# IseanB/SensorFusion-KalmanFilter

Hardware: AMD Instinct MI355X
Metric: KF predict+update steps/sec (batched filters) (higher is better)
Workload: dtype f64

## Files before the change

### include/kf.h

```cpp
#ifndef KFMI_KF_H
#define KFMI_KF_H

#include <stdint.h>

#ifdef __cplusplus
extern "C" {
#endif

#define KF_OK        0
#define KF_EINVAL   (-1)
#define KF_EHIP     (-2)
#define KF_ENOTSPD  (-3)
#define KF_ENODEV   (-4)
#define KF_ENOMEM   (-5)

#define KF_F32 0
#define KF_F64 1

#define KF_MODEL_CV2 2
#define KF_MODEL_CV3 3

#define KF_MODEL_REF15 15

#define KF_MODEL_REF8 8
// ... 76 lines not shown

int kf_run_events(kf_batch* handle, int T, const uint8_t* etype, const double* dt, const void* payload,
                  void* traj, void* cov, void* logdet, uint8_t* updated, int gate, double threshold,
                  void* stream);

int kf_run_events_seq(kf_batch* handle, int T, const uint8_t* etype, const double* dt, const void* payload,
                      void* traj, void* cov, void* logdet, uint8_t* updated, int gate, double threshold,
                      void* stream);

int kf_run_events_gates(kf_batch* handle, int T, const uint8_t* etype, const double* dt, const void* payload,
                        void* traj, void* cov, void* logdet, uint8_t* updated, const double* thresholds,
                        void* stream);

int kf_run_stream(kf_batch* handle, int T, const uint8_t* etype, const double* dt, const void* payload,
                  void* traj, void* cov, void* logdet, uint8_t* updated, int chunk, int warmup,
                  void* stream);

int kf_run_sweep(kf_batch* handle, int T, const uint8_t* etype, const double* dt, const void* payload,
                 const double* thresholds, void* traj, void* logdet, uint8_t* updated, int32_t* n_updated,
                 int ckpt_every, void* ckpt_x, void* ckpt_P, void* stream);

int kf_stream_check(kf_batch* handle, double* out, void* stream);

int kf_eval_combos(kf_batch* handle, int n_events, const double* events, const double* init,
                   double prev_time, double target_end, int k, uint64_t combo_offset, void* logdets,
                   void* max_logdet, int32_t* n_records, void* stream);

int kf_search_combos(kf_batch* handle, int n_events, const double* events, const double* init,
                     double prev_time, double target_end, double threshold, int k_max, int exhaustive,
                     int n_fixed, uint64_t fixed_mask, uint64_t* winner, int* k_found,
                     uint64_t* n_accepted, void* subset_max, void* stream);

int kf_search_windows(kf_batch* handle, int W, int n_max, const int32_t* n_events, const double* events,
                      const double* init, const double* prev_time, const double* target_end,
                      const double* threshold, int k_max, uint64_t* winner, int32_t* k_found,
                      uint64_t* n_accepted, void* stream);

int kf_search_plan(const kf_batch* handle, int n_events, const double* init, int n_fixed, uint64_t fixed_mask,
                   int k_max, int64_t* out);

int kf_search_info(const kf_batch* handle, int64_t* out);

int kf_score_candidates(kf_batch* handle, int n_types, const int32_t* types, int full, void* gain,
                        void* post, void* stream);

int kf_score_rows(kf_batch* handle, int n_cand, const int32_t* types, const uint32_t* row_masks, void* gain,
// ... 58 lines not shown
```

### sensorfusion-kalmanfilter_amd/csrc/kf_capi.cpp

```cpp
#include <hip/hip_runtime.h>

#include <algorithm>
#include <cmath>
#include <climits>
#include <cstdarg>
#include <cstdlib>
#include <cstdio>
#include <cstring>
#include <mutex>
#include <string>
#include <vector>

#include "../../include/kf.h"
#include "kf_internal.h"

struct kf_batch {
    int model;
    int axes;
    int n, m, c;
    int np;
    int dtype;
    int64_t B;
    int device;
    kf_params params;
// ... 47 lines not shown

thread_local std::string g_err;

int fail(int code, const char* fmt, ...) __attribute__((format(printf, 2, 3)));
int fail(int code, const char* fmt, ...) {
    char buf[512];
    va_list ap;
    va_start(ap, fmt);
    vsnprintf(buf, sizeof buf, fmt, ap);
    va_end(ap);
    g_err = buf;
    return code;
}

int hip_fail(hipError_t e, const char* what) {
    return fail(KF_EHIP, "%s: %s (%d)", what, hipGetErrorString(e), static_cast<int>(e));
}

size_t elem(const kf_batch* h) { return h->dtype == KF_F64 ? 8 : 4; }
int64_t ntri(const kf_batch* h) { return h->np; }

constexpr int kMaxComboEvents = 64;
constexpr int64_t kChainMaxFilters = 16384;
constexpr size_t kWsEvents = sizeof(double) * kMaxComboEvents * 11;
constexpr size_t kWsBinom = sizeof(uint64_t) * (kMaxComboEvents + 1) * (kMaxComboEvents + 1);
constexpr size_t kWsInit = sizeof(double) * 42;
constexpr uint64_t kSearchChildMajorParents = 200000;
constexpr uint64_t kSearchHeadSteps = 400000;
constexpr uint64_t kSearchEndSteps = 200000;
constexpr uint64_t kSearchPairParents = uint64_t(1) << 22;

int64_t opt(const kf_batch* h, int o) { return h->opt[o]; }

bool is_ref15(const kf_batch* h) { return h->model == KF_MODEL_REF15; }

const uint64_t* binom_table() {
    static uint64_t binom[(kMaxComboEvents + 1) * (kMaxComboEvents + 1)];
    static std::once_flag once;
    std::call_once(once, [] {
        for (int a = 0; a <= kMaxComboEvents; ++a)
            for (int b = 0; b <= kMaxComboEvents; ++b) {
                uint64_t v = 0;
                if (b == 0) v = 1;
                else if (a > 0 && b <= a) v = binom[(a - 1) * (kMaxComboEvents + 1) + b - 1] + binom[(a - 1) * (kMaxComboEvents + 1) + b];
                binom[a * (kMaxComboEvents + 1) + b] = v;
            }
// ... 625 lines not shown
    if (int rc = need_cv(h, "kf_synth")) return rc;
    if (T < 0 || update_every < 1 || filter_offset < 0)
        return fail(KF_EINVAL, "kf_synth: bad T/update_every/filter_offset");
    if (h->B && (!x0_out || (T > 0 && !u_out) || (T / update_every > 0 && !z_out)))
        return fail(KF_EINVAL, "kf_synth: null output stream");
    if (h->B == 0) return KF_OK;
    kfmi::SynthArgs a{};
    a.B = h->B;
    a.filter_offset = filter_offset;
    a.seed = seed;
    a.T = T;
    a.update_every = update_every;
    a.dt = dt;
    a.x0 = x0_out;
    a.u = u_out;
    a.z = z_out;
    hipError_t e = kfmi::launch_synth(h->axes, h->dtype == KF_F64, a, static_cast<hipStream_t>(stream));
    if (e != hipSuccess) return hip_fail(e, "kf_synth");
    return KF_OK;
}

namespace {

int run_events_launch(kf_batch* h, int T, const uint8_t* etype, const double* dt, const void* payload, void* traj,
                      void* cov, void* logdet, uint8_t* updated, int gate, double threshold, const int32_t* skip,
                      void* stream, int forced = -1, const double* thresholds = nullptr) {
    kfmi::RefArgs a = ref_args(h);
    a.thresholds = thresholds;
    a.T = T;
    a.etype = etype;
    a.dt = dt;
    a.payload = payload;
    a.traj = traj;
    a.cov = cov;
    a.logdet = logdet;
    a.updated = updated;
    a.gate = gate;
    a.threshold = threshold;
    a.skip = skip;
    const uint64_t span = static_cast<uint64_t>(h->B) * elem(h);
    const bool chain_ok = span * 27u < (uint64_t(1) << 32);
    const bool lds_ok = h->B % 16 == 0 && span * 9u < (uint64_t(1) << 32);
    int variant = h->B < kChainMaxFilters && chain_ok ? kfmi::kEventsChain
                  : lds_ok                            ? kfmi::kEventsLds
                                                      : kfmi::kEventsLane;
    const int64_t v = opt(h, KF_OPT_EVENTS_KERNEL);
    if (v == 2 && chain_ok) variant = kfmi::kEventsChain;
    else if (v == 1) variant = kfmi::kEventsLane;
    else if (v == 3 && lds_ok) variant = kfmi::kEventsLds;
    else if (v == 4 && h->B == 1 && gate && h->dtype == KF_F64) variant = kfmi::kEventsGated;
    if (forced >= 0) variant = forced;
    if (skip && variant != kfmi::kEventsChain && variant != kfmi::kEventsGated)
        return fail(KF_EINVAL, "kf_run_stream: fallback needs the chain kernel");
    hipError_t e = kfmi::launch_ref_events(h->model, h->dtype == KF_F64, a, static_cast<hipStream_t>(stream), variant);
    return e == hipSuccess ? KF_OK : hip_fail(e, "kf_run_events");
}

constexpr int kStreamMinEvents = 65536;
constexpr int kStreamGateWarmup = 2048;
constexpr int kStreamLookaheadShare = 8;
constexpr int64_t kStreamLftEvents = 2048;
constexpr int kStreamPolish = 0;
constexpr int64_t kStreamLftPiece = 160;
constexpr int64_t kStreamTargetChunks = 8192;
constexpr int64_t kStreamMinChunk = 32;
constexpr int64_t kStreamStartLdsMaps = 65536 / (36 * 8);
#ifndef KF_START_MAX_G
#define KF_START_MAX_G 2
#endif

size_t align256(size_t n) { return (n + 255) & ~size_t(255); }

}

namespace {
// ... 262 lines not shown
    } else {
        if (e == hipSuccess) e = chain(C, sa.mx, sa.mP, sa.mst, L, 0, false, nullptr, 1, 4);
        for (int ph : {kfmi::kStreamPhaseScanTiles, kfmi::kStreamPhaseTop, kfmi::kStreamPhaseStarts})
            if (e == hipSuccess && (ph != kfmi::kStreamPhaseTop || top))
                e = kfmi::launch_stream_phase(h->model, f64, ph, sa, st);
        if (e == hipSuccess) e = chain(C, sa.fx, sa.fP, sa.fst, L, 0, true);
        if (e == hipSuccess) e = kfmi::launch_stream_phase(h->model, f64, kfmi::kStreamPhaseFinish, sa, st);
    }
    if (e != hipSuccess) return hip_fail(e, "kf_run_stream");
    if (gate && f64 && updated && opt(h, KF_OPT_EVENTS_KERNEL) == 0) {
        e = kfmi::launch_stream_choose(sa.check, updated, T, kStreamLookaheadShare, st);
        if (e != hipSuccess) return hip_fail(e, "kf_run_stream");
        int rc = run_events_launch(h, T, etype, dt, payload, traj, cov, logdet, updated, gate, threshold,
                                   &sa.check->skip_gated, stream, kfmi::kEventsGated);
        if (rc != KF_OK) return rc;
        return run_events_launch(h, T, etype, dt, payload, traj, cov, logdet, updated, gate, threshold,
                                 &sa.check->skip_chain, stream, kfmi::kEventsChain);
    }
    return run_events_launch(h, T, etype, dt, payload, traj, cov, logdet, updated, gate, threshold, &sa.check->ok,
                             stream);
}
}

int kf_stream_check(kf_batch* h, double* out, void* stream) {
    if (int rc = check_handle(h)) return rc;
    if (!out) return fail(KF_EINVAL, "kf_stream_check: null output");
    if (!h->stream_ws && h->s_chunks != 1) return fail(KF_EINVAL, "kf_stream_check: no kf_run_stream on this handle");
    kfmi::StreamCheck k{};
    if (h->s_chunks > 1) {
        hipError_t e = hipMemcpyAsync(&k, h->stream_ws, sizeof k, hipMemcpyDeviceToHost, static_cast<hipStream_t>(stream));
        if (e == hipSuccess) e = hipStreamSynchronize(static_cast<hipStream_t>(stream));
        if (e != hipSuccess) return hip_fail(e, "kf_stream_check");
    }
    out[0] = k.ok;
    out[1] = (k.bad & ~kfmi::kStreamBadStart) ? 1.0 : 0.0;
    out[2] = k.cov_gap;
    out[3] = k.state_gap;
    out[4] = double(h->s_chunks);
    out[5] = double(h->s_len);
    out[6] = double(h->s_warm);
    out[7] = h->s_chunks > 1 && k.ok ? 0.0 : k.skip_chain ? 4.0 : 2.0;
    return KF_OK;
}

int kf_eval_combos(kf_batch* h, int n_events, const double* events, const double* init, double prev_time,
                   double target_end, int k, uint64_t combo_offset, void* logdets, void* max_logdet,
// ... 636 lines not shown
```

### sensorfusion-kalmanfilter_amd/csrc/kf_common.h

```cpp
#pragma once

#include <hip/hip_runtime.h>
#include <math.h>
#include <stdint.h>

namespace kfmi {
namespace dev {

constexpr int32_t kNotSpd = -3;

template <int N>
__host__ __device__ constexpr int tri(int i, int j) {
    return i <= j ? i * N - i * (i - 1) / 2 + (j - i) : j * N - j * (j - 1) / 2 + (i - j);
}

__device__ __forceinline__ double fmaT(double a, double b, double c) { return __builtin_fma(a, b, c); }
__device__ __forceinline__ float fmaT(float a, float b, float c) { return __builtin_fmaf(a, b, c); }

template <typename T>
__device__ __forceinline__ T quiet_nan();
template <>
__device__ __forceinline__ double quiet_nan<double>() { return __builtin_nan(""); }
template <>
__device__ __forceinline__ float quiet_nan<float>() { return __builtin_nanf(""); }
// ... 91 lines not shown
template <typename T>
__device__ __forceinline__ void det2(const T (&P)[3], T& num, bool& ok) {
    const T m2 = fmaT(-P[1], P[1], P[0] * P[2]);
    ok = ok && (P[0] > T(0)) && (m2 > T(0));
    num *= m2;
}
template <typename T>
__device__ __forceinline__ void renorm(T& prod, int& ex) {
    int e;
    prod = frexp(prod, &e);
    ex += e;
}

template <int N, typename T>
__device__ __forceinline__ T logdet_ldl(const T (&P)[N * (N + 1) / 2]) {
    T prod = T(1);
    int ex = 0;
    bool ok = true;
    ldl_pivot_product<N, T>(P, prod, ex, ok);
    const T ld = log_mant(prod, ex);
    return ok ? ld : quiet_nan<T>();
}

template <int N, int M, bool DIAG_R, typename T, int NEWTON = 2, bool POISON = true, int NV = 1, bool JOSEPH = true,
          bool GAIN_R = false>
__device__ __forceinline__ bool sel_update_nv(T (&xv)[NV][N], T (&P)[N * (N + 1) / 2], const T (&zv)[NV][M],
                                              const T (&R)[M * (M + 1) / 2]) {
    constexpr int MT = M * (M + 1) / 2;
    T S[MT];
#pragma unroll
    for (int i = 0; i < M; ++i)
#pragma unroll
        for (int j = i; j < M; ++j)
            S[tri<M>(i, j)] = (i == j || !DIAG_R) ? P[tri<N>(i, j)] + R[tri<M>(i, j)] : P[tri<N>(i, j)];
    T L[M][M];
    T d[M];
    T dinv[M];
    bool ok = true;
#pragma unroll
    for (int j = 0; j < M; ++j) {
        T v[M];
        T dj = S[tri<M>(j, j)];
#pragma unroll
        for (int k = 0; k < j; ++k) {
            v[k] = L[j][k] * d[k];
            dj = fmaT(-L[j][k], v[k], dj);
        }
        ok = ok && (dj > T(0));
        d[j] = dj;
        dinv[j] = POISON ? rcp_pos<NEWTON>(dj) : rcp_nr<NEWTON>(dj);
#pragma unroll
        for (int i = j + 1; i < M; ++i) {
            T s = S[tri<M>(i, j)];
#pragma unroll
            for (int k = 0; k < j; ++k) s = fmaT(-L[i][k], v[k], s);
            L[i][j] = s * dinv[j];
        }
    }
    T K[N][M];
#pragma unroll
    for (int i = 0; i < N; ++i) {
        T w[M];
#pragma unroll
        for (int a = 0; a < M; ++a) {
            T s = P[tri<N>(i, a)];
#pragma unroll
            for (int b = 0; b < a; ++b) s = fmaT(-L[a][b], w[b], s);
            w[a] = s;
        }
#pragma unroll
        for (int a = M - 1; a >= 0; --a) {
            T s = w[a] * dinv[a];
#pragma unroll
            for (int b = a + 1; b < M; ++b) s = fmaT(-L[b][a], K[i][b], s);
            K[i][a] = s;
        }
    }
#pragma unroll
    for (int v = 0; v < NV; ++v) {
        T y[M];
#pragma unroll
        for (int a = 0; a < M; ++a) y[a] = zv[v][a] - xv[v][a];
#pragma unroll
        for (int i = 0; i < N; ++i) {
            T s = xv[v][i];
#pragma unroll
            for (int a = 0; a < M; ++a) s = fmaT(K[i][a], y[a], s);
            xv[v][i] = s;
        }
    }
    if constexpr (GAIN_R && M == N && DIAG_R) {
#pragma unroll
        for (int i = 0; i < N; ++i)
#pragma unroll
            for (int j = i; j < N; ++j) P[tri<N>(i, j)] = K[i][j] * R[tri<M>(j, j)];
        return ok;
    }
    T top[M][N];
#pragma unroll
    for (int i = 0; i < N; ++i) {
        T E[M];
        if constexpr (JOSEPH) {
#pragma unroll
            for (int a = 0; a < M; ++a) {
                T e = -P[tri<N>(i, a)];
#pragma unroll
                for (int b = 0; b < M; ++b) e = fmaT(K[i][b], S[tri<M>(b, a)], e);
                E[a] = e;
            }
        }
#pragma unroll
        for (int j = i; j < N; ++j) {
            T s = P[tri<N>(i, j)];
#pragma unroll
            for (int b = 0; b < M; ++b) s = fmaT(-K[i][b], P[tri<N>(b, j)], s);
            if constexpr (JOSEPH) {
#pragma unroll
                for (int a = 0; a < M; ++a) s = fmaT(E[a], K[j][a], s);
            }
            if (i < M)
                top[i][j] = s;
            else
                P[tri<N>(i, j)] = s;
        }
    }
#pragma unroll
    for (int i = 0; i < M; ++i)
#pragma unroll
        for (int j = i; j < N; ++j) P[tri<N>(i, j)] = top[i][j];
    return ok;
}

template <int N, int M, bool DIAG_R, typename T, int NEWTON = 2, bool POISON = true, bool JOSEPH = true,
          bool GAIN_R = false>
__device__ __forceinline__ bool sel_update(T (&x)[N], T (&P)[N * (N + 1) / 2], const T (&z)[M],
                                           const T (&R)[M * (M + 1) / 2]) {
    T xv[1][N], zv[1][M];
#pragma unroll
    for (int i = 0; i < N; ++i) xv[0][i] = x[i];
#pragma unroll
    for (int a = 0; a < M; ++a) zv[0][a] = z[a];
    const bool ok = sel_update_nv<N, M, DIAG_R, T, NEWTON, POISON, 1, JOSEPH, GAIN_R>(xv, P, zv, R);
#pragma unroll
    for (int i = 0; i < N; ++i) x[i] = xv[0][i];
    return ok;
}

typedef unsigned int v2u __attribute__((ext_vector_type(2)));

__device__ __forceinline__ __amdgpu_buffer_rsrc_t row_rsrc(const void* base, int64_t r, uint32_t row_bytes) {
    const char* p = reinterpret_cast<const char*>(base) + r * int64_t(row_bytes);
    return __builtin_amdgcn_make_buffer_rsrc(const_cast<char*>(p), 0, row_bytes, 0x00020000);
}
// ... 131 lines not shown
```

### sensorfusion-kalmanfilter_amd/csrc/kf_internal.h

```cpp
#pragma once

#include <hip/hip_runtime.h>
#include <stdint.h>

namespace kfmi {

struct CvArgs {
    int64_t B;
    int T;
    int update_every;
    double dt;
    const double* dt_steps;
    const double* dt_filter;
    void* x;
    void* P;
    int32_t* status;
    const void* u;
    const void* x0;
    const void* z;
    const uint8_t* mask;
    void* traj;
    void* logdet;
    double q_pos, q_vel;
    double r[6];
// ... 254 lines not shown
    int gps_wins;
    bool fused;
    int group_waves;
    bool one_launch;
    uint32_t* wave_key;
    uint32_t* wave_id;
    uint32_t* wave_key_sorted;
    uint32_t* order;
    void* sort_tmp;
    size_t sort_tmp_bytes;
    const uint32_t* words;
    int n_words;
    int32_t* words_used;
    bool rec_time;
};

enum class Op { Run, Predict, Update, Step, Reset };

hipError_t launch_cv(int axes, bool f64, Op op, const CvArgs& a, hipStream_t stream);
hipError_t launch_cv_offblock(int axes, bool f64, const CvArgs& a, int* flag, hipStream_t stream);
hipError_t launch_synth(int axes, bool f64, const SynthArgs& a, hipStream_t stream);
hipError_t launch_copy(void* dst, const void* src, size_t bytes, hipStream_t stream);
constexpr int kEventsLane = 0, kEventsChain = 1, kEventsLds = 2, kEventsGated = 3;
hipError_t launch_ref_events(int model, bool f64, const RefArgs& a, hipStream_t stream, int variant);
hipError_t launch_ref_stream(int model, bool f64, const RefArgs& a, hipStream_t stream, int nv = 1);
hipError_t launch_ref_sweep(int model, bool f64, const SweepArgs& a, hipStream_t stream);
hipError_t launch_ref_reset(int model, bool f64, const RefArgs& a, hipStream_t stream);
hipError_t launch_ref15_combos(bool f64, const Ref15ComboArgs& a, hipStream_t stream);
hipError_t launch_ref15_search(bool f64, const Ref15SearchArgs& a, bool child_major, hipStream_t stream);
hipError_t launch_ref15_search_pair(bool f64, const Ref15SearchArgs& a, bool child_major, hipStream_t stream);
void set_search_band(Ref15SearchArgs& a, bool f64);
hipError_t launch_ref15_search_head(bool f64, const Ref15SearchArgs& a, hipStream_t stream);
hipError_t launch_ref15_search_end(bool f64, const Ref15SearchArgs& a, hipStream_t stream);
hipError_t launch_ref15_search_windows(bool f64, bool sym, const Ref15WindowArgs* wins, int W, uint64_t max_lanes,
                                       int n_max, int k_max, const uint64_t* binom, const RefConsts* kc,
                                       hipStream_t stream);
hipError_t launch_search_windows_finish(const Ref15WindowArgs* wins, int W, int k_max, uint64_t* host,
                                        hipStream_t stream);
hipError_t launch_search_finish(uint64_t* counters, uint64_t* host, int n, bool zero, hipStream_t stream);
hipError_t launch_ref15_score(bool f64, const Ref15ScoreArgs& a, hipStream_t stream);
hipError_t launch_ref15_scheduled(bool f64, const Ref15SchedArgs& a, hipStream_t stream);
hipError_t launch_ref15_random_picks(const Ref15SchedArgs& a, int32_t* pick, hipStream_t stream);
hipError_t sort_pairs_desc_u32(void* tmp, size_t* tmp_bytes, const uint32_t* keys_in, uint32_t* keys_out,
                               const uint32_t* vals_in, uint32_t* vals_out, int n, int bits, hipStream_t stream);

constexpr int kBlock = 256;
// ... 5 lines not shown
```

### sensorfusion-kalmanfilter_amd/csrc/kf_ref.hip

```cpp
#include <hip/hip_runtime.h>
#include <stdint.h>

#include <cmath>
#include <cstdlib>
#include <cstring>

#include "kf_common.h"
#include "kf_internal.h"

namespace kfmi {
namespace {

template <typename T>
__device__ __forceinline__ __attribute__((address_space(4))) const T* ro(const T* p) {
    return (__attribute__((address_space(4))) const T*)p;
}
typedef __attribute__((address_space(4))) const double ro_double;
typedef __attribute__((address_space(4))) const uint64_t ro_u64;

using namespace dev;

constexpr int kGps = 0, kImu = 1;
constexpr int kRefNewton = 1;
#ifndef KF_REF_JOSEPH_F64
#define KF_REF_JOSEPH_F64 0
#endif
template <typename T>
constexpr bool kRefJoseph = sizeof(T) == 4 || KF_REF_JOSEPH_F64 != 0;
// ... 941 lines not shown
                    gap = fmax(gap, fabs(pe - wnx[k]));
                }
                const double rel = gap / fmax(scale, 1e-300);
                crel = rel == rel ? rel : __builtin_inf();
            }
        }
        if (a.s_check) {
            crel = fmax(crel, dpp_d<kDppXor1>(crel));
            crel = fmax(crel, dpp_d<kDppXor2>(crel));
            crel = fmax(crel, dpp_d<kDppHalfMirror>(crel));
            const bool full = (g & ~int64_t(63)) / LPF + 64 / LPF <= a.B;
            if (full) {
#pragma unroll
                for (int sh = kGroup; sh < 64; sh <<= 1) crel = fmax(crel, __shfl_xor(crel, sh, 64));
                const bool lane0 = (threadIdx.x & 63) == 0;
                if (lane0 && crel != 0.0) atomic_max_pos(&a.s_check->cov_gap, crel);
                const bool any_bad = __builtin_amdgcn_ballot_w64(c == 0 && st != 0) != 0;
                if (lane0 && any_bad) atomicOr(&a.s_check->bad, kStreamBadFilter);
            } else {
                if (c == 0 && vb == 0 && crel != 0.0) atomic_max_pos(&a.s_check->cov_gap, crel);
                if (c == 0 && vb == 0 && st != 0) atomicOr(&a.s_check->bad, kStreamBadFilter);
            }
        }
    }
}

#ifndef KF_SWEEP_DEPTH
#define KF_SWEEP_DEPTH 4
#endif
constexpr int kSweepDepth = KF_SWEEP_DEPTH;
constexpr int kSweepBlock = 64;

template <typename T, class M, bool CUSTOM>
__global__ __launch_bounds__(kSweepBlock) void ref_sweep_kernel(const SweepArgs a) {
    const int64_t g = static_cast<int64_t>(blockIdx.x) * kSweepBlock + threadIdx.x;
    const int64_t f = g / kGroup;
    if (f >= a.B) return;
    const int c = static_cast<int>(g % kGroup);
    const bool pva = c < M::NP;
    const bool live = c < M::NP + M::NA;
    const int ca = pva ? c : (live ? c - M::NP : 0);
    const uint32_t off = uint32_t(f) * uint32_t(sizeof(T));
    const uint32_t rb = uint32_t(a.B) * uint32_t(sizeof(T));
    int xi[3], pr[6];
#pragma unroll
    for (int k = 0; k < 3; ++k) xi[k] = !live ? -1 : pva ? M::pva(ca, k) : (k < 2 ? M::aw(ca, k) : -1);
// ... 2970 lines not shown
    KF_CUSTOM_DISPATCH(a.kc, {
        if (lds) {
            if (f64) ref15_sched_lds_kernel<double, CUSTOM><<<grid, kBlock, 0, stream>>>(a);
            else ref15_sched_lds_kernel<float, CUSTOM><<<grid, kBlock, 0, stream>>>(a);
        } else {
            if (f64) ref15_sched_kernel<double, CUSTOM><<<grid, kBlock, 0, stream>>>(a);
            else ref15_sched_kernel<float, CUSTOM><<<grid, kBlock, 0, stream>>>(a);
        }
    });
    return hipGetLastError();
}

namespace {
template <typename T, class M, bool CUSTOM>
void ref_events_t(const RefArgs& a, hipStream_t stream, int variant) {
    if (a.thresholds) {
        if (variant == kEventsLds) {
            const dim3 grid(static_cast<unsigned>((a.B + kBlock - 1) / kBlock));
            if (a.cov) ref_events_lds_kernel<T, M, true, CUSTOM, true><<<grid, kBlock, 0, stream>>>(a);
            else ref_events_lds_kernel<T, M, false, CUSTOM, true><<<grid, kBlock, 0, stream>>>(a);
        } else if (variant == kEventsChain) {
            const dim3 cgrid(static_cast<unsigned>((a.B * kGroup + kBlock - 1) / kBlock));
            ref_chain_kernel<T, M, false, CUSTOM, 1, true><<<cgrid, kBlock, 0, stream>>>(a);
        } else {
            const dim3 grid(static_cast<unsigned>((a.B + kBlock - 1) / kBlock));
            ref_events_kernel<T, M, CUSTOM, true><<<grid, kBlock, 0, stream>>>(a);
        }
        return;
    }
    if (variant == kEventsLds) {
        const dim3 grid(static_cast<unsigned>((a.B + kBlock - 1) / kBlock));
        if (a.cov) ref_events_lds_kernel<T, M, true, CUSTOM><<<grid, kBlock, 0, stream>>>(a);
        else ref_events_lds_kernel<T, M, false, CUSTOM><<<grid, kBlock, 0, stream>>>(a);
    } else if (variant == kEventsChain) {
        const dim3 cgrid(static_cast<unsigned>((a.B * kGroup + kBlock - 1) / kBlock));
        ref_chain_kernel<T, M, false, CUSTOM><<<cgrid, kBlock, 0, stream>>>(a);
    } else if (variant == kEventsGated) {
        ref_chain_gated_kernel<T, M, CUSTOM><<<1, 64, 0, stream>>>(a);
    } else {
        const dim3 grid(static_cast<unsigned>((a.B + kBlock - 1) / kBlock));
        ref_events_kernel<T, M, CUSTOM><<<grid, kBlock, 0, stream>>>(a);
    }
}
template <typename T, class M, bool CUSTOM>
void ref_stream_t(const RefArgs& a, hipStream_t stream, int nv) {
    if (nv == 4) {
        const dim3 vgrid(static_cast<unsigned>((a.B * chain_lanes<4>() + kBlock - 1) / kBlock));
        ref_chain_kernel<T, M, true, CUSTOM, 4><<<vgrid, kBlock, 0, stream>>>(a);
    } else {
        const dim3 cgrid(static_cast<unsigned>((a.B * kGroup + kBlock - 1) / kBlock));
        ref_chain_kernel<T, M, true, CUSTOM><<<cgrid, kBlock, 0, stream>>>(a);
    }
}
}

hipError_t launch_ref_events(int model, bool f64, const RefArgs& a, hipStream_t stream, int variant) {
    if (model != 15 && model != 8) return hipErrorInvalidValue;
    if (a.thresholds && (variant == kEventsGated || a.s_len != 0)) return hipErrorInvalidValue;
    KF_CUSTOM_DISPATCH(a.kc, {
// ... 349 lines not shown
```

### sensorfusion-kalmanfilter_amd/kfmi/_lib.py

```python
from __future__ import annotations

import ctypes
import glob
import hashlib
import os
import re

HERE = os.path.dirname(os.path.abspath(__file__))
LIB_PATH = os.path.abspath(os.environ.get('KFMI_LIB') or os.path.join(HERE, 'libkfmi.so'))
HEADER = os.path.normpath(os.path.join(HERE, '..', '..', 'include', 'kf.h'))
CSRC = os.path.normpath(os.path.join(HERE, '..', 'csrc'))

KF_OK = 0
KF_EINVAL = -1
KF_EHIP = -2
KF_ENOTSPD = -3
KF_ENODEV = -4
KF_ENOMEM = -5
KF_F32 = 0
KF_F64 = 1
KF_MODEL_CV2 = 2
KF_MODEL_CV3 = 3
KF_MODEL_REF15 = 15
KF_MODEL_REF8 = 8
# ... 63 lines not shown
    'kf_last_error': (ctypes.c_char_p, []),
    'kf_default_params': (_i, [_i, ctypes.POINTER(kf_params)]),
    'kf_device_count': (_i, [ctypes.POINTER(_i)]),
    'kf_init': (_i, [_i]),
    'kf_alloc': (_i, [ctypes.POINTER(_vp), _i, _i64, _i, ctypes.POINTER(kf_params)]),
    'kf_free': (_i, [_vp]),
    'kf_release_retired': (_i, [_vp, ctypes.POINTER(_i64)]),
    'kf_dims': (_i, [_vp, ctypes.POINTER(_i), ctypes.POINTER(_i), ctypes.POINTER(_i),
                     ctypes.POINTER(_i64), ctypes.POINTER(_i)]),
    'kf_reset': (_i, [_vp, _vp, _vp]),
    'kf_set_state': (_i, [_vp, _vp, _vp, _i, _vp]),
    'kf_get_state': (_i, [_vp, _vp, _vp, _i, _vp]),
    'kf_get_status': (_i, [_vp, _vp, _i, _vp]),
    'kf_predict': (_i, [_vp, _d, _vp, _vp, _vp, _vp]),
    'kf_update': (_i, [_vp, _vp, _vp, _vp, _vp]),
    'kf_run': (_i, [_vp, _i, _d, _vp, _vp, _vp, _vp, _i, _vp, _vp, _vp]),
    'kf_synth': (_i, [_vp, ctypes.c_uint64, _i64, _i, _d, _i, _vp, _vp, _vp, _vp]),
    'kf_run_events': (_i, [_vp, _i, _vp, _vp, _vp, _vp, _vp, _vp, _vp, _i, _d, _vp]),
    'kf_run_events_seq': (_i, [_vp, _i, _vp, _vp, _vp, _vp, _vp, _vp, _vp, _i, _d, _vp]),
    'kf_run_events_gates': (_i, [_vp, _i, _vp, _vp, _vp, _vp, _vp, _vp, _vp, _vp, _vp]),
    'kf_run_stream': (_i, [_vp, _i, _vp, _vp, _vp, _vp, _vp, _vp, _vp, _i, _i, _vp]),
    'kf_run_sweep': (_i, [_vp, _i, _vp, _vp, _vp, _vp, _vp, _vp, _vp, _vp, _i, _vp, _vp, _vp]),
    'kf_stream_check': (_i, [_vp, _vp, _vp]),
    'kf_eval_combos': (_i, [_vp, _i, _vp, _vp, _d, _d, _i, ctypes.c_uint64, _vp, _vp, _vp, _vp]),
    'kf_search_combos': (_i, [_vp, _i, _vp, _vp, _d, _d, _d, _i, _i, _i, ctypes.c_uint64,
                              ctypes.POINTER(ctypes.c_uint64), ctypes.POINTER(_i), _vp, _vp, _vp]),
    'kf_search_windows': (_i, [_vp, _i, _i, _vp, _vp, _vp, _vp, _vp, _vp, _i, _vp, _vp, _vp, _vp]),
    'kf_search_plan': (_i, [_vp, _i, _vp, _i, ctypes.c_uint64, _i, _vp]),
    'kf_search_info': (_i, [_vp, _vp]),
    'kf_score_candidates': (_i, [_vp, _i, _vp, _i, _vp, _vp, _vp]),
    'kf_score_rows': (_i, [_vp, _i, _vp, _vp, _vp, _vp, _vp]),
    'kf_run_scheduled': (_i, [_vp, _i, _vp, _vp, _vp, _vp, _vp, _d, _vp, _vp, _vp, _vp, _vp]),
    'kf_run_scheduled_rec': (_i, [_vp, _i, _vp, _vp, _vp, _i, _vp, _vp, _d, _vp, _vp, _vp, _vp, _vp]),
    'kf_run_scheduled_random': (_i, [_vp, _i, _vp, _vp, _vp, _i, _vp, _vp, _d, _vp, _i, _vp, _vp, _vp, _vp, _vp,
                                     _vp]),
    'kf_sched_random_picks': (_i, [_vp, _i, _vp, _vp, _vp, _vp, _d, _vp, _i, _vp, _vp, _vp, _vp, _vp]),
    'kf_csv_shape': (_i, [ctypes.c_char_p, _i, ctypes.POINTER(_i64), ctypes.POINTER(_i)]),
    'kf_csv_read': (_i, [ctypes.c_char_p, _i, _i, _vp, _i64, _i64]),
    'kf_ingest': (_i, [_vp, _i64, _i64, _vp, _i64, _i64, _i, _vp, _vp, _vp, _vp, _vp, _vp, _vp,
                       ctypes.POINTER(kf_ingest_info), _vp]),
    'kf_quat_to_euler': (_i, [_i64, _vp, _i64, _vp, _vp]),
    'kf_events_dt': (_i, [_i64, _vp, _vp, _d, _i, _vp, _vp, _vp]),
    'kf_events_select': (_i, [_i64, _vp, _vp, _vp, _i, _vp, _vp, _vp, ctypes.POINTER(_i64), _vp]),
}

_lib = None
# ... 71 lines not shown
```

### sensorfusion-kalmanfilter_amd/kfmi/engine.py

```python
from __future__ import annotations

import ctypes

import numpy as np
import torch

from . import _lib
from ._lib import KFError, check

MODELS = {
    'cv2': (_lib.KF_MODEL_CV2, 4, 2, 2, 10),
    'cv3': (_lib.KF_MODEL_CV3, 6, 3, 3, 21),
    'ref15': (_lib.KF_MODEL_REF15, 15, 3, 0, 27),
    'ref8': (_lib.KF_MODEL_REF8, 8, 2, 0, 15),
}
REF_MODELS = ('ref15', 'ref8')
TRAJ_WIDTH = {'ref15': 6, 'ref8': 3}
DTYPES = {'f32': (_lib.KF_F32, torch.float32, np.float32), 'f64': (_lib.KF_F64, torch.float64, np.float64)}


OPTIONS = {
    'predict': (_lib.KF_OPT_PREDICT, {'auto': 0, 'deferred': 0, 'eager': 1}),
    'cv_kernel': (_lib.KF_OPT_CV_KERNEL, {'auto': 0, 'general': 1, 'block2': 2, 'block4': 4, 'block8': 8}),
    'blocks_per_cu': (_lib.KF_OPT_BLOCKS_PER_CU, {'auto': 0}),
# ... 319 lines not shown
                  checkpoint_every=0):
        if self.model not in REF_MODELS:
            raise ValueError('run_sweep needs a ref15 or ref8 handle')
        T = int(etype.shape[0])
        every = int(checkpoint_every)
        if every < 0:
            raise ValueError('checkpoint_every must be >= 0')
        et = self._dev(etype.reshape(T), (T,), 'etype', torch.uint8)
        dtd = self._dev(dt.reshape(T), (T,), 'dt', torch.float64)
        pay = self._dev(payload.reshape(T, 9), (T, 9), 'payload')
        thr = self._dev(thresholds, (self.batch,), 'thresholds', torch.float64)
        tr = self.empty(T, TRAJ_WIDTH[self.model], self.batch) if traj else None
        ld = self.empty(T, self.batch) if logdet else None
        up = torch.empty(T, self.batch, dtype=torch.uint8, device=self.device) if updated else None
        nu = torch.zeros(self.batch, dtype=torch.int32, device=self.device) if counts else None
        C = T // every if every > 0 else 0
        cx = self.empty(C, self.n, self.batch) if every > 0 else None
        cP = self.empty(C, self.ntri, self.batch) if every > 0 else None
        check(_lib.lib().kf_run_sweep(self.handle, T, _ptr(et), _ptr(dtd), _ptr(pay), _ptr(thr), _ptr(tr), _ptr(ld),
                                      _ptr(up), _ptr(nu), every, _ptr(cx) if C else None, _ptr(cP) if C else None,
                                      self._stream()))
        return tr, ld, up, nu, cx, cP

    def stream_check(self):
        out = (ctypes.c_double * 8)()
        check(_lib.lib().kf_stream_check(self.handle, out, self._stream()))
        return dict(ok=bool(out[0]), failed_chunk=bool(out[1]), cov_gap=out[2], state_gap=out[3],
                    chunks=int(out[4]), chunk=int(out[5]), warmup=int(out[6]),
                    fallback={0: None, 2: 'chain', 4: 'gated'}[int(out[7])])

    def eval_combos(self, events, init, prev_time, target_end, k, combo_offset=0, logdets=True):
        if self.model != 'ref15':
            raise ValueError('eval_combos needs a ref15 handle')
        ev = np.ascontiguousarray(events, dtype=np.float64)
        ini = np.ascontiguousarray(init, dtype=np.float64)
        if ev.ndim != 2 or ev.shape[1] != 11 or ini.shape != (42,):
            raise ValueError('events must be [n, 11] and init [42]')
        mx = self.empty(self.batch)
        ld = self.empty(k + 2, self.batch) if logdets else None
        nr = torch.empty(self.batch, dtype=torch.int32, device=self.device)
        check(_lib.lib().kf_eval_combos(self.handle, ev.shape[0], ev.ctypes.data_as(ctypes.c_void_p),
                                        ini.ctypes.data_as(ctypes.c_void_p), float(prev_time), float(target_end),
                                        int(k), int(combo_offset), _ptr(ld), _ptr(mx), _ptr(nr), self._stream()))
        torch.cuda.current_stream(self.device).synchronize()
        return mx, ld, nr

# ... 187 lines not shown
```

Baseline: 57.45 billion.

## Add warp-specialized split chain kernel for small-batch event runs

Adds a new events kernel for batches of up to 4096 filters. One wave runs the covariance predict and gain computation, a second wave applies the gains to the state and writes the records, and an optional third wave computes log-determinants. The waves hand gains and covariances to each other through double-buffered LDS in batches of events, so the serial covariance chain overlaps with state updates and output stores. This costs block-wide barriers per batch, 64 KB of static LDS per block, and fewer filters per block. The headline metric is for batched filters and may run at a batch size that never reaches this path.

```diff
diff --git a/include/kf.h b/include/kf.h
--- a/include/kf.h
+++ b/include/kf.h
@@ -122,6 +122,8 @@
 
 int kf_stream_check(kf_batch* handle, double* out, void* stream);
 
+int kf_events_kernel(const kf_batch* handle, int gate, int* kernel);
+
 int kf_eval_combos(kf_batch* handle, int n_events, const double* events, const double* init,
                    double prev_time, double target_end, int k, uint64_t combo_offset, void* logdets,
                    void* max_logdet, int32_t* n_records, void* stream);
diff --git a/sensorfusion-kalmanfilter_amd/csrc/kf_capi.cpp b/sensorfusion-kalmanfilter_amd/csrc/kf_capi.cpp
--- a/sensorfusion-kalmanfilter_amd/csrc/kf_capi.cpp
+++ b/sensorfusion-kalmanfilter_amd/csrc/kf_capi.cpp
@@ -93,6 +93,7 @@
 
 constexpr int kMaxComboEvents = 64;
 constexpr int64_t kChainMaxFilters = 16384;
+constexpr int64_t kSplitMaxFilters = 4096;
 constexpr size_t kWsEvents = sizeof(double) * kMaxComboEvents * 11;
 constexpr size_t kWsBinom = sizeof(uint64_t) * (kMaxComboEvents + 1) * (kMaxComboEvents + 1);
 constexpr size_t kWsInit = sizeof(double) * 42;
@@ -764,6 +765,23 @@
 
 namespace {
 
+int events_variant(const kf_batch* h, int gate, int forced) {
+    const uint64_t span = static_cast<uint64_t>(h->B) * elem(h);
+    const bool chain_ok = span * 27u < (uint64_t(1) << 32);
+    const bool lds_ok = h->B % 16 == 0 && span * 9u < (uint64_t(1) << 32);
+    int variant = h->B < kChainMaxFilters && chain_ok ? kfmi::kEventsChain
+                  : lds_ok                            ? kfmi::kEventsLds
+                                                      : kfmi::kEventsLane;
+    const int64_t v = opt(h, KF_OPT_EVENTS_KERNEL);
+    if (v == 2 && chain_ok) variant = kfmi::kEventsChain;
+    else if (v == 1) variant = kfmi::kEventsLane;
+    else if (v == 3 && lds_ok) variant = kfmi::kEventsLds;
+    else if (v == 4 && h->B == 1 && gate && h->dtype == KF_F64) variant = kfmi::kEventsGated;
+    if (forced >= 0) variant = forced;
+    if (v != 2 && variant == kfmi::kEventsChain && h->B <= kSplitMaxFilters) variant = kfmi::kEventsSplit;
+    return variant;
+}
+
 int run_events_launch(kf_batch* h, int T, const uint8_t* etype, const double* dt, const void* payload, void* traj,
                       void* cov, void* logdet, uint8_t* updated, int gate, double threshold, const int32_t* skip,
                       void* stream, int forced = -1, const double* thresholds = nullptr) {
@@ -780,19 +798,8 @@
     a.gate = gate;
     a.threshold = threshold;
     a.skip = skip;
-    const uint64_t span = static_cast<uint64_t>(h->B) * elem(h);
-    const bool chain_ok = span * 27u < (uint64_t(1) << 32);
-    const bool lds_ok = h->B % 16 == 0 && span * 9u < (uint64_t(1) << 32);
-    int variant = h->B < kChainMaxFilters && chain_ok ? kfmi::kEventsChain
-                  : lds_ok                            ? kfmi::kEventsLds
-                                                      : kfmi::kEventsLane;
-    const int64_t v = opt(h, KF_OPT_EVENTS_KERNEL);
-    if (v == 2 && chain_ok) variant = kfmi::kEventsChain;
-    else if (v == 1) variant = kfmi::kEventsLane;
-    else if (v == 3 && lds_ok) variant = kfmi::kEventsLds;
-    else if (v == 4 && h->B == 1 && gate && h->dtype == KF_F64) variant = kfmi::kEventsGated;
-    if (forced >= 0) variant = forced;
-    if (skip && variant != kfmi::kEventsChain && variant != kfmi::kEventsGated)
+    const int variant = events_variant(h, gate, forced);
+    if (skip && variant != kfmi::kEventsChain && variant != kfmi::kEventsSplit && variant != kfmi::kEventsGated)
         return fail(KF_EINVAL, "kf_run_stream: fallback needs the chain kernel");
     hipError_t e = kfmi::launch_ref_events(h->model, h->dtype == KF_F64, a, static_cast<hipStream_t>(stream), variant);
     return e == hipSuccess ? KF_OK : hip_fail(e, "kf_run_events");
@@ -1101,6 +1108,20 @@
 }
 }
 
+int kf_events_kernel(const kf_batch* h, int gate, int* kernel) {
+    if (int rc = check_handle(h)) return rc;
+    if (!is_ref(h)) return fail(KF_EINVAL, "kf_events_kernel: needs a KF_MODEL_REF15 or KF_MODEL_REF8 handle");
+    if (!kernel) return fail(KF_EINVAL, "kf_events_kernel: null output");
+    switch (events_variant(h, gate, -1)) {
+        case kfmi::kEventsLane: *kernel = 1; break;
+        case kfmi::kEventsChain: *kernel = 2; break;
+        case kfmi::kEventsLds: *kernel = 3; break;
+        case kfmi::kEventsGated: *kernel = 4; break;
+        default: *kernel = 5; break;
+    }
+    return KF_OK;
+}
+
 int kf_stream_check(kf_batch* h, double* out, void* stream) {
     if (int rc = check_handle(h)) return rc;
     if (!out) return fail(KF_EINVAL, "kf_stream_check: null output");
diff --git a/sensorfusion-kalmanfilter_amd/csrc/kf_common.h b/sensorfusion-kalmanfilter_amd/csrc/kf_common.h
--- a/sensorfusion-kalmanfilter_amd/csrc/kf_common.h
+++ b/sensorfusion-kalmanfilter_amd/csrc/kf_common.h
@@ -137,10 +137,13 @@
     return ok ? ld : quiet_nan<T>();
 }
 
-template <int N, int M, bool DIAG_R, typename T, int NEWTON = 2, bool POISON = true, int NV = 1, bool JOSEPH = true,
-          bool GAIN_R = false>
-__device__ __forceinline__ bool sel_update_nv(T (&xv)[NV][N], T (&P)[N * (N + 1) / 2], const T (&zv)[NV][M],
-                                              const T (&R)[M * (M + 1) / 2]) {
+struct SelNoApply {
+    __device__ __forceinline__ void operator()() const {}
+};
+template <int N, int M, bool DIAG_R, typename T, int NEWTON = 2, bool POISON = true, bool JOSEPH = true,
+          bool GAIN_R = false, class Apply = SelNoApply>
+__device__ __forceinline__ bool sel_gain(T (&P)[N * (N + 1) / 2], const T (&R)[M * (M + 1) / 2], T (&K)[N][M],
+                                         const Apply& with_gain = Apply()) {
     constexpr int MT = M * (M + 1) / 2;
     T S[MT];
 #pragma unroll
@@ -172,7 +175,6 @@
             L[i][j] = s * dinv[j];
         }
     }
-    T K[N][M];
 #pragma unroll
     for (int i = 0; i < N; ++i) {
         T w[M];
@@ -191,19 +193,7 @@
             K[i][a] = s;
         }
     }
-#pragma unroll
-    for (int v = 0; v < NV; ++v) {
-        T y[M];
-#pragma unroll
-        for (int a = 0; a < M; ++a) y[a] = zv[v][a] - xv[v][a];
-#pragma unroll
-        for (int i = 0; i < N; ++i) {
-            T s = xv[v][i];
-#pragma unroll
-            for (int a = 0; a < M; ++a) s = fmaT(K[i][a], y[a], s);
-            xv[v][i] = s;
-        }
-    }
+    with_gain();
     if constexpr (GAIN_R && M == N && DIAG_R) {
 #pragma unroll
         for (int i = 0; i < N; ++i)
@@ -244,6 +234,32 @@
 #pragma unroll
         for (int j = i; j < N; ++j) P[tri<N>(i, j)] = top[i][j];
     return ok;
+}
+
+template <int N, int M, typename T, int NV = 1>
+__device__ __forceinline__ void sel_apply(T (&xv)[NV][N], const T (&zv)[NV][M], const T (&K)[N][M]) {
+#pragma unroll
+    for (int v = 0; v < NV; ++v) {
+        T y[M];
+#pragma unroll
+        for (int a = 0; a < M; ++a) y[a] = zv[v][a] - xv[v][a];
+#pragma unroll
+        for (int i = 0; i < N; ++i) {
+            T s = xv[v][i];
+#pragma unroll
+            for (int a = 0; a < M; ++a) s = fmaT(K[i][a], y[a], s);
+            xv[v][i] = s;
+        }
+    }
+}
+
+template <int N, int M, bool DIAG_R, typename T, int NEWTON = 2, bool POISON = true, int NV = 1, bool JOSEPH = true,
+          bool GAIN_R = false>
+__device__ __forceinline__ bool sel_update_nv(T (&xv)[NV][N], T (&P)[N * (N + 1) / 2], const T (&zv)[NV][M],
+                                              const T (&R)[M * (M + 1) / 2]) {
+    T K[N][M];
+    return sel_gain<N, M, DIAG_R, T, NEWTON, POISON, JOSEPH, GAIN_R>(P, R, K,
+                                                                     [&]() { sel_apply<N, M, T, NV>(xv, zv, K); });
 }
 
 template <int N, int M, bool DIAG_R, typename T, int NEWTON = 2, bool POISON = true, bool JOSEPH = true,
diff --git a/sensorfusion-kalmanfilter_amd/csrc/kf_internal.h b/sensorfusion-kalmanfilter_amd/csrc/kf_internal.h
--- a/sensorfusion-kalmanfilter_amd/csrc/kf_internal.h
+++ b/sensorfusion-kalmanfilter_amd/csrc/kf_internal.h
@@ -300,6 +300,7 @@
 hipError_t launch_synth(int axes, bool f64, const SynthArgs& a, hipStream_t stream);
 hipError_t launch_copy(void* dst, const void* src, size_t bytes, hipStream_t stream);
 constexpr int kEventsLane = 0, kEventsChain = 1, kEventsLds = 2, kEventsGated = 3;
+constexpr int kEventsSplit = 4;
 hipError_t launch_ref_events(int model, bool f64, const RefArgs& a, hipStream_t stream, int variant);
 hipError_t launch_ref_stream(int model, bool f64, const RefArgs& a, hipStream_t stream, int nv = 1);
 hipError_t launch_ref_sweep(int model, bool f64, const SweepArgs& a, hipStream_t stream);
diff --git a/sensorfusion-kalmanfilter_amd/csrc/kf_ref.hip b/sensorfusion-kalmanfilter_amd/csrc/kf_ref.hip
--- a/sensorfusion-kalmanfilter_amd/csrc/kf_ref.hip
+++ b/sensorfusion-kalmanfilter_amd/csrc/kf_ref.hip
@@ -4,6 +4,7 @@
 #include <cmath>
 #include <cstdlib>
 #include <cstring>
+#include <type_traits>
 
 #include "kf_common.h"
 #include "kf_internal.h"
@@ -991,6 +992,302 @@
                 if (c == 0 && vb == 0 && st != 0) atomicOr(&a.s_check->bad, kStreamBadFilter);
             }
         }
+    }
+}
+
+#ifndef KF_SPLIT_BATCH
+#define KF_SPLIT_BATCH 4
+#endif
+constexpr int kSplitBatch = KF_SPLIT_BATCH;
+constexpr int kSplitSlots = 16;
+constexpr int kSplitBlock = 192;
+static_assert(2 * kSplitBatch * kSplitSlots * 64 * 8 <= 65536, "the two hand-off buffers: 64 KB of static LDS in f64");
+
+template <typename T, class M, bool CUSTOM, bool COV, bool GATES = false>
+__global__ __launch_bounds__(kSplitBlock) void ref_chain_split_kernel(const RefArgs a) {
+    if (a.T <= 0 || (a.skip && *a.skip)) return;
+    constexpr int R = kSplitBatch;
+    constexpr int kSlot = kSplitSlots * 64;
+    __shared__ __attribute__((aligned(16))) T hand[2 * R * kSlot];
+    const int lane = int(threadIdx.x & 63u);
+    const int role = wave_uniform(int(threadIdx.x >> 6));
+    const bool leader = role == 0;
+    const int64_t g = static_cast<int64_t>(blockIdx.x) * 64 + lane;
+    const bool dead = g / kGroup >= a.B;
+    const int64_t f = dead ? a.B - 1 : g / kGroup;
+    const int c = static_cast<int>(g % kGroup);
+    const bool pva = c < M::NP && !dead;
+    const bool live = c < M::NP + M::NA && !dead;
+    const int ca = pva ? c : (live ? c - M::NP : 0);
+    const uint32_t off = uint32_t(f) * uint32_t(sizeof(T));
+    const uint32_t rb = uint32_t(a.B) * uint32_t(sizeof(T));
+    const uint32_t rb8 = uint32_t(a.B) * 8u;
+    const uint32_t off8 = uint32_t(f) * 8u;
+    int xi[3], pr[6];
+#pragma unroll
+    for (int k = 0; k < 3; ++k) xi[k] = !live ? -1 : pva ? M::pva(ca, k) : (k < 2 ? M::aw(ca, k) : -1);
+#pragma unroll
+    for (int k = 0; k < 6; ++k) {
+        const int aw_row = k == 0 ? 0 : k == 1 ? 1 : k == 3 ? 2 : -1;
+        pr[k] = !live ? -1 : pva ? 6 * ca + k : (aw_row < 0 ? -1 : 6 * M::NP + 3 * ca + aw_row);
+    }
+    uint32_t vx[3], vp[6];
+#pragma unroll
+    for (int k = 0; k < 3; ++k) vx[k] = xi[k] >= 0 ? uint32_t(xi[k]) * rb + off : kDropOffset;
+#pragma unroll
+    for (int k = 0; k < 6; ++k) vp[k] = pr[k] >= 0 ? uint32_t(pr[k]) * rb + off : kDropOffset;
+    const uint32_t v_tr = (xi[0] >= 0 && xi[0] < M::NTRAJ) ? uint32_t(xi[0]) * rb + off : kDropOffset;
+    const bool first = c == 0 && !dead;
+    const uint32_t v_ld = first ? off : kDropOffset;
+    const int ia = pva ? ca : M::imu_att(ca);
+    const int ib = pva ? M::imu_acc(ca) : M::imu_rate(ca);
+    const uint32_t v_a = uint32_t(ia) * rb + off, v_b = uint32_t(ib) * rb + off;
+    T q[3] = {T(pva ? kQPos : kQAtt), T(pva ? kQVel : kQRate), T(pva ? kQAcc : 0.0)};
+    T Rimu[6] = {T(pva ? kRPos : kRAtt), T(0), T(0), T(pva ? kRVel : kRRate), T(0), T(pva ? kRAcc : 1.0)};
+    T Rgps = T(kRGps);
+    if constexpr (CUSTOM) {
+        const RefConsts* kc = a.kc;
+#pragma unroll
+        for (int k = 0; k < 3; ++k)
+            if (xi[k] >= 0) {
+                q[k] = T(ro(kc)->q[xi[k]]);
+                Rimu[k == 0 ? 0 : k == 1 ? 3 : 5] = T(ro(kc)->r_imu[xi[k]]);
+            }
+        if (pva) Rgps = T(ro(kc)->r_gps[ca]);
+    }
+
+    const auto rx = span_rsrc(a.x, 0, rb, M::N), rp = span_rsrc(a.P, 0, rb, M::NBLK);
+    T x[1][3], P[6];
+#pragma unroll
+    for (int k = 0; k < 3; ++k) x[0][k] = ldv(rx, vx[k], T(0));
+#pragma unroll
+    for (int k = 0; k < 6; ++k) P[k] = pr[k] >= 0 ? ldv(rp, vp[k], T(0)) : T(k == 0 || k == 3 || k == 5 ? 1 : 0);
+    bool failed = false;
+    const bool need_ld = a.logdet != nullptr;
+    const bool need_P = need_ld || COV;
+    GateBand<T> gate;
+    FilterGate<T> fg{false, T(0)};
+    if constexpr (GATES) {
+        fg = gate_of<T>(a.thresholds, f);
+        if (fg.on) gate.init(a.thresholds[f]);
+    } else {
+        if (a.gate) gate.init(a.threshold);
+    }
+
+    const int T_ = a.T;
+    struct Batch {
+        ChainIn<T> e[R];
+    };
+    auto load_batch = [&](int b, Batch& in, auto with_payload) {
+#pragma unroll
+        for (int j = 0; j < R; ++j) {
+            const int t = b * R + j < T_ ? b * R + j : T_ - 1;
+            in.e[j].type = int(ldb<uint8_t>(a.etype, t, uint32_t(a.B), uint32_t(f)));
+            in.e[j].dt = ldb<double>(a.dt, t, rb8, off8);
+            in.e[j].va = in.e[j].vb = T(0);
+            if constexpr (decltype(with_payload)::value) {
+                const auto rpay = span_rsrc(a.payload, int64_t(t) * 9, rb, 9);
+                in.e[j].va = ldv(rpay, v_a, T(0));
+                in.e[j].vb = ldv(rpay, v_b, T(0));
+            }
+        }
+    };
+    auto lead = [&](const ChainIn<T>& in, T* hs) {
+        const int type = in.type;
+        const T dt = T(in.dt);
+        int flags = 0;
+        if (type != 255) {
+            const T c02 = pva ? T(0.5) * dt * dt : T(0);
+            const T c12 = pva ? dt : T(0);
+            T FP[3][3];
+#pragma unroll
+            for (int j = 0; j < 3; ++j) {
+                FP[0][j] = fmaT(c02, P[tri<3>(2, j)], fmaT(dt, P[tri<3>(1, j)], P[tri<3>(0, j)]));
+                FP[1][j] = fmaT(c12, P[tri<3>(2, j)], P[tri<3>(1, j)]);
+                FP[2][j] = P[tri<3>(2, j)];
+            }
+#pragma unroll
+            for (int i = 0; i < 3; ++i)
+#pragma unroll
+                for (int j = i; j < 3; ++j) {
+                    T s = FP[i][j];
+                    if (j == 0) s = fmaT(FP[i][2], c02, fmaT(FP[i][1], dt, s));
+                    if (j == 1) s = fmaT(FP[i][2], c12, s);
+                    P[tri<3>(i, j)] = (i == j) ? s + q[i] * dt : s;
+                }
+            bool applied = (type == kGps || type == kImu);
+            if constexpr (GATES) {
+                if (fg.on && applied) applied = gate.open(P, live, fg.thr);
+            } else {
+                if (a.gate && applied) applied = gate.open(P, live, T(a.threshold));
+            }
+            bool ok = true;
+            if (applied) {
+                if (type == kGps) {
+                    if (pva) {
+                        T K[3][1];
+                        const T Rg[1] = {Rgps};
+                        ok = sel_gain<3, 1, true, T, kRefNewton, true, kRefJoseph<T>, kRefGainR>(P, Rg, K);
+#pragma unroll
+                        for (int i = 0; i < 3; ++i) hs[i * 64] = K[i][0];
+                    }
+                } else {
+                    T K[3][3];
+                    ok = sel_gain<3, 3, true, T, kRefNewton, true, kRefJoseph<T>, kRefGainR>(P, Rimu, K);
+#pragma unroll
+                    for (int i = 0; i < 3; ++i)
+#pragma unroll
+                        for (int m = 0; m < 3; ++m) hs[(3 * i + m) * 64] = K[i][m];
+                    if (!pva) P[5] = T(1);
+                }
+            }
+            const bool bad = group_any(!ok);
+            if (bad) {
+#pragma unroll
+                for (int k = 0; k < 6; ++k) P[k] = quiet_nan<T>();
+            }
+            flags = (applied ? 1 : 0) | (bad ? 2 : 0);
+        }
+        *reinterpret_cast<int*>(hs + 15 * 64) = flags;
+        if (need_P) {
+#pragma unroll
+            for (int k = 0; k < 6; ++k) hs[(9 + k) * 64] = P[k];
+        }
+    };
+    const char* p_tr = static_cast<const char*>(a.traj);
+    const char* p_cv = static_cast<const char*>(a.cov);
+    const char* p_ld = static_cast<const char*>(a.logdet);
+    const char* p_up = reinterpret_cast<const char*>(a.updated);
+    const uint32_t n_tr = a.traj ? rb * uint32_t(M::NTRAJ) : 0u, n_cv = a.cov ? rb * uint32_t(M::NBLK) : 0u;
+    const uint32_t n_ld = a.logdet ? rb : 0u, n_up = a.updated ? uint32_t(a.B) : 0u;
+    auto rec_rsrc = [](const char* base, uint32_t nbytes) {
+        return __builtin_amdgcn_make_buffer_rsrc(const_cast<char*>(base), 0, nbytes, 0x00020000);
+    };
+    auto follow = [&](const ChainIn<T>& in, const T* hs) {
+        const int type = in.type;
+        const T dt = T(in.dt);
+        const T va = in.va, vb = in.vb;
+        const int flags = *reinterpret_cast<const int*>(hs + 15 * 64);
+        const bool applied = (flags & 1) != 0;
+        if (type != 255) {
+            const T c02 = pva ? T(0.5) * dt * dt : T(0);
+            const T c12 = pva ? dt : T(0);
+            const T xn0 = fmaT(c02, x[0][2], fmaT(dt, x[0][1], x[0][0]));
+            const T xn1 = fmaT(c12, x[0][2], x[0][1]);
+            x[0][0] = xn0;
+            x[0][1] = xn1;
+            if (applied) {
+                if (type == kGps) {
+                    if (pva) {
+                        T K[3][1];
+#pragma unroll
+                        for (int i = 0; i < 3; ++i) K[i][0] = hs[i * 64];
+                        const T zb[1][1] = {{va}};
+                        sel_apply<3, 1, T, 1>(x, zb, K);
+                    }
+                } else {
+                    T zb[1][3];
+                    const T V = fmaT(vb, dt, x[0][1]);
+                    const T X = fmaT(V, dt, x[0][0]);
+                    zb[0][0] = pva ? X : va;
+                    zb[0][1] = pva ? V : vb;
+                    zb[0][2] = pva ? vb : T(0);
+                    T K[3][3];
+#pragma unroll
+                    for (int i = 0; i < 3; ++i)
+#pragma unroll
+                        for (int m = 0; m < 3; ++m) K[i][m] = hs[(3 * i + m) * 64];
+                    sel_apply<3, 3, T, 1>(x, zb, K);
+                    if (!pva) x[0][2] = T(0);
+                }
+            }
+            if (flags & 2) {
+                failed = true;
+#pragma unroll
+                for (int k = 0; k < 3; ++k) x[0][k] = quiet_nan<T>();
+            }
+        }
+        stv(rec_rsrc(p_tr, n_tr), v_tr, x[0][0]);
+        p_tr += size_t(rb) * M::NTRAJ;
+        if constexpr (COV) {
+            const auto rc = rec_rsrc(p_cv, n_cv);
+#pragma unroll
+            for (int k = 0; k < 6; ++k) stv(rc, vp[k], hs[(9 + k) * 64]);
+            p_cv += size_t(rb) * M::NBLK;
+        }
+        __builtin_amdgcn_raw_buffer_store_b8(applied ? uint8_t(1) : uint8_t(0), rec_rsrc(p_up, n_up),
+                                             first ? uint32_t(f) : kDropOffset, 0, 0);
+        p_up += a.B;
+    };
+    auto log_det = [&](const T* hs) {
+        T Pe[6];
+#pragma unroll
+        for (int k = 0; k < 6; ++k) Pe[k] = hs[(9 + k) * 64];
+        const T ld = group_sum(live ? chain_log_det(Pe) : T(0));
+        failed = failed || !(ld == ld);
+        stv(rec_rsrc(p_ld, n_ld), v_ld, ld);
+        p_ld += rb;
+    };
+
+    const int NBf = T_ / R;
+    const bool tail = NBf * R < T_;
+    auto slot = [&](int b, int j) { return hand + (b & 1) * (R * kSlot) + j * kSlot + lane; };
+    Batch cur, nxt;
+    if (leader) {
+        load_batch(0, cur, std::false_type());
+        for (int b = 0; b < NBf; ++b) {
+            load_batch(b + 1, nxt, std::false_type());
+#pragma unroll
+            for (int j = 0; j < R; ++j) lead(cur.e[j], slot(b, j));
+            __syncthreads();
+            cur = nxt;
+        }
+        if (tail) {
+#pragma unroll
+            for (int j = 0; j < R - 1; ++j)
+                if (NBf * R + j < T_) lead(cur.e[j], slot(NBf, j));
+            __syncthreads();
+        }
+        __syncthreads();
+#pragma unroll
+        for (int k = 0; k < 6; ++k) stv(rp, vp[k], P[k]);
+    } else if (role == 2) {
+        __syncthreads();
+        for (int b = 0; b < NBf; ++b) {
+            if (need_ld) {
+#pragma unroll
+                for (int j = 0; j < R; ++j) log_det(slot(b, j));
+            }
+            __syncthreads();
+        }
+        if (tail) {
+            if (need_ld) {
+#pragma unroll
+                for (int j = 0; j < R - 1; ++j)
+                    if (NBf * R + j < T_) log_det(slot(NBf, j));
+            }
+            __syncthreads();
+        }
+        if (first && failed) a.status[f] = kNotSpd;
+    } else {
+        load_batch(0, cur, std::true_type());
+        __syncthreads();
+        for (int b = 0; b < NBf; ++b) {
+            load_batch(b + 1, nxt, std::true_type());
+#pragma unroll
+            for (int j = 0; j < R; ++j) follow(cur.e[j], slot(b, j));
+            __syncthreads();
+            cur = nxt;
+        }
+        if (tail) {
+#pragma unroll
+            for (int j = 0; j < R - 1; ++j)
+                if (NBf * R + j < T_) follow(cur.e[j], slot(NBf, j));
+            __syncthreads();
+        }
+#pragma unroll
+        for (int k = 0; k < 3; ++k) stv(rx, vx[k], x[0][k]);
+        if (first && failed) a.status[f] = kNotSpd;
     }
 }
 
@@ -4007,6 +4304,11 @@
         } else if (variant == kEventsChain) {
             const dim3 cgrid(static_cast<unsigned>((a.B * kGroup + kBlock - 1) / kBlock));
             ref_chain_kernel<T, M, false, CUSTOM, 1, true><<<cgrid, kBlock, 0, stream>>>(a);
+        } else if (variant == kEventsSplit) {
+            const dim3 sgrid(static_cast<unsigned>((a.B + kGroup - 1) / kGroup));
+            const int sblock = a.logdet ? kSplitBlock : kSplitBlock - 64;
+            if (a.cov) ref_chain_split_kernel<T, M, CUSTOM, true, true><<<sgrid, sblock, 0, stream>>>(a);
+            else ref_chain_split_kernel<T, M, CUSTOM, false, true><<<sgrid, sblock, 0, stream>>>(a);
         } else {
             const dim3 grid(static_cast<unsigned>((a.B + kBlock - 1) / kBlock));
             ref_events_kernel<T, M, CUSTOM, true><<<grid, kBlock, 0, stream>>>(a);
@@ -4020,6 +4322,11 @@
     } else if (variant == kEventsChain) {
         const dim3 cgrid(static_cast<unsigned>((a.B * kGroup + kBlock - 1) / kBlock));
         ref_chain_kernel<T, M, false, CUSTOM><<<cgrid, kBlock, 0, stream>>>(a);
+    } else if (variant == kEventsSplit) {
+        const dim3 sgrid(static_cast<unsigned>((a.B + kGroup - 1) / kGroup));
+        const int sblock = a.logdet ? kSplitBlock : kSplitBlock - 64;
+        if (a.cov) ref_chain_split_kernel<T, M, CUSTOM, true><<<sgrid, sblock, 0, stream>>>(a);
+        else ref_chain_split_kernel<T, M, CUSTOM, false><<<sgrid, sblock, 0, stream>>>(a);
     } else if (variant == kEventsGated) {
         ref_chain_gated_kernel<T, M, CUSTOM><<<1, 64, 0, stream>>>(a);
     } else {
diff --git a/sensorfusion-kalmanfilter_amd/kfmi/_lib.py b/sensorfusion-kalmanfilter_amd/kfmi/_lib.py
--- a/sensorfusion-kalmanfilter_amd/kfmi/_lib.py
+++ b/sensorfusion-kalmanfilter_amd/kfmi/_lib.py
@@ -109,6 +109,7 @@
     'kf_run_stream': (_i, [_vp, _i, _vp, _vp, _vp, _vp, _vp, _vp, _vp, _i, _i, _vp]),
     'kf_run_sweep': (_i, [_vp, _i, _vp, _vp, _vp, _vp, _vp, _vp, _vp, _vp, _i, _vp, _vp, _vp]),
     'kf_stream_check': (_i, [_vp, _vp, _vp]),
+    'kf_events_kernel': (_i, [_vp, _i, ctypes.POINTER(_i)]),
     'kf_eval_combos': (_i, [_vp, _i, _vp, _vp, _d, _d, _i, ctypes.c_uint64, _vp, _vp, _vp, _vp]),
     'kf_search_combos': (_i, [_vp, _i, _vp, _vp, _d, _d, _d, _i, _i, _i, ctypes.c_uint64,
                               ctypes.POINTER(ctypes.c_uint64), ctypes.POINTER(_i), _vp, _vp, _vp]),
diff --git a/sensorfusion-kalmanfilter_amd/kfmi/engine.py b/sensorfusion-kalmanfilter_amd/kfmi/engine.py
--- a/sensorfusion-kalmanfilter_amd/kfmi/engine.py
+++ b/sensorfusion-kalmanfilter_amd/kfmi/engine.py
@@ -365,6 +365,11 @@
                                       self._stream()))
         return tr, ld, up, nu, cx, cP
 
+    def events_kernel(self, gate=False):
+        out = ctypes.c_int(0)
+        check(_lib.lib().kf_events_kernel(self.handle, int(bool(gate)), ctypes.byref(out)))
+        return {1: 'lane', 2: 'chain', 3: 'lds', 4: 'gated', 5: 'split'}[out.value]
+
     def stream_check(self):
         out = (ctypes.c_double * 8)()
         check(_lib.lib().kf_stream_check(self.handle, out, self._stream()))
```

After: 54.33 billion. -5.4%, worse.
